# TEAM-AIOLY/OCM-VAE-SIMCA

Measured on AMD Instinct MI355X. Metric: spectra/sec SIMCA fit+Q/T² score at 1M×2048, higher is better.
Workload: dtype f32

## Files before the change

### ocm-vae-simca_amd/csrc/ocm_gram.hip

```cpp
#include <cstring>
#include <string>
#include <vector>

#include "ocm_internal.h"

namespace {

__device__ __forceinline__ float load_y(const float* __restrict__ X, int64_t ldx, int64_t r, int col, int p,
                                        const PrepArgs& pa) {
  if (pa.w == 0 && !pa.snv) return X[r * ldx + col];
  float m = 0.f, sc = 1.f;
  if (pa.snv) {
    m = pa.rowstat[2 * r];
    sc = pa.rowstat[2 * r + 1];
  }
  return ocm::prep_elem(X + r * ldx, p, col, pa, m, sc);
}


constexpr int MAXSEG = 32;

struct SegTable {
  int64_t begin[MAXSEG + 1];
  int32_t cprefix[MAXSEG + 1];
  int32_t nseg;
  int32_t chunk_rows;
};

__device__ __forceinline__ void tile_coords(int t, int nt, int& ti, int& tj) {
  ti = 0;
  while (t >= nt - ti) {
    t -= nt - ti;
    ++ti;
  }
  tj = ti + t;
}

template <int GT, int BK_>
struct GramCfg {
  static constexpr int BK = BK_;
  static constexpr int WN = GT / 64;
  static constexpr int THREADS = 2 * WN * 64;
  static constexpr int MT = GT / 64;
  static constexpr int C4 = GT / 4;
  static constexpr int RSTEP = THREADS / C4;
  static constexpr int LPP = BK / RSTEP;
};

constexpr int GATHER_MAX_CHUNK = 2048;

template <int GT, int BK_, bool VEC, bool GATHER>
__global__ __launch_bounds__(GT * 2, 2) void k_gram(
    const float* __restrict__ X, int64_t ldx, const int64_t* __restrict__ rows, int p, const float* __restrict__ shift,
    SegTable st, int nt, int ntiles, int total_wg, float* __restrict__ part, double* __restrict__ colpart) {
  using Cfg = GramCfg<GT, BK_>;
  constexpr int BK = Cfg::BK, MT = Cfg::MT, LPP = Cfg::LPP, RSTEP = Cfg::RSTEP;
// ... 1224 lines not shown
  const int tid = threadIdx.x, tx = tid & 15, ty = tid >> 4;
  const int gI = I / Q8GROUP, gJ = J / Q8GROUP;
  double acc[4][4] = {};
  for (int64_t f0 = fa; f0 < fb; f0 += FX_R) {
    const int nr = (int)min<int64_t>(FX_R, fb - f0);
    __syncthreads();
    for (int e = tid; e < FX_R * FX_T; e += 256) {
      const int r = e / FX_T, c = e % FX_T;
      double a = 0.0, b = 0.0;
      if (r < nr) {
        const int64_t pos = list[f0 + r];
        const int64_t xrow = rows ? rows[pos] : pos;
        if (I + c < p) a = (double)load_y(X, ldx, xrow, I + c, p, pa) - (double)shift[I + c];
        if (J + c < p) b = (double)load_y(X, ldx, xrow, J + c, p, pa) - (double)shift[J + c];
      }
      yi[r][c] = a;
      yj[r][c] = b;
    }
    if (tid < FX_R) {
      uint32_t m = 0;
      if (tid < nr) {
        const int64_t pos = list[f0 + tid];
        auto bit = [&](int g) { return (flags[(size_t)pos * fw + (g >> 5)] >> (g & 31)) & 1u; };
        m = bit(gI) | (bit(gI + 1) << 1) | (bit(gJ) << 2) | (bit(gJ + 1) << 3);
      }
      mk[tid] = m;
    }
    __syncthreads();
    for (int r = 0; r < nr; ++r) {
      const uint32_t m = mk[r];
      const bool mi = (m >> (ty >> 3)) & 1u;
      const bool mj = (m >> (2 + (tx >> 3))) & 1u;
      if (!(mi || mj)) continue;
#pragma unroll
      for (int a = 0; a < 4; ++a) {
        const double u = yi[r][4 * ty + a];
#pragma unroll
        for (int b = 0; b < 4; ++b) acc[a][b] = fma(u, yj[r][4 * tx + b], acc[a][b]);
      }
    }
  }
  double* Gs = G + (size_t)seg * p * p;
#pragma unroll
  for (int a = 0; a < 4; ++a)
#pragma unroll
    for (int b = 0; b < 4; ++b) {
      const int gi = I + 4 * ty + a, gj = J + 4 * tx + b;
      if (gi >= p || gj >= p) continue;
      Gs[(size_t)gi * p + gj] += acc[a][b];
      if (ti != tj) Gs[(size_t)gj * p + gi] += acc[a][b];
    }
}

#ifndef OCM_G8_BAND_R
#define OCM_G8_BAND_R 4
#endif
#ifndef OCM_G8_BAND_C
#define OCM_G8_BAND_C 8
#endif
constexpr int G8_BAND_R = OCM_G8_BAND_R, G8_BAND_C = OCM_G8_BAND_C;
__global__ __launch_bounds__(256, 1) void k_gram8d(Q8Plan q, SegTable st, int nt, int ntiles, int total_wg,
                                                   int nwg, int nblocks, float* __restrict__ part) {
  __shared__ __attribute__((aligned(16))) float scl[4][2 * 64];
  __shared__ __attribute__((aligned(16))) float runl[4][4][4][64][4];

  const int b = blockIdx.x;
  const int q8 = total_wg / 8, r8 = total_wg % 8, x8 = b % 8;
  const int wg = (x8 < r8 ? x8 * (q8 + 1) : r8 * (q8 + 1) + (x8 - r8) * q8) + b / 8;
  const int chunk = wg / nwg;
  const int wave = __builtin_amdgcn_readfirstlane(threadIdx.x >> 6);
  const int bi = (wg - chunk * nwg) * 4 + wave;
  if (bi >= nblocks) return;
  int ti = -1, tj = 0, wm = 0, wn = 0;
  {
    int rem = bi;
    for (int u = 0; u < nt && ti < 0; u += G8_BAND_R)
      for (int v = u; v < nt && ti < 0; v += G8_BAND_C)
        for (int a = u; a < min(nt, u + G8_BAND_R) && ti < 0; ++a)
          for (int c = max(v, a); c < min(nt, v + G8_BAND_C); ++c) {
            const int nbk = (a == c) ? 3 : 4;
            if (rem < nbk) {
              ti = a;
              tj = c;
              wm = (a == c) ? (rem == 2) : (rem >> 1);
              wn = (a == c) ? (rem >= 1) : (rem & 1);
              break;
            }
            rem -= nbk;
          }
  }
  const int tile = ti * nt - ti * (ti - 1) / 2 + (tj - ti);
  const int I = ti * Q8T, J = tj * Q8T;
  int s = 0;
  while (s + 1 < st.nseg && chunk >= st.cprefix[s + 1]) ++s;
  const int64_t r0 = st.begin[s] + (int64_t)(chunk - st.cprefix[s]) * st.chunk_rows;
  const int64_t r1 = min(r0 + (int64_t)st.chunk_rows, st.begin[s + 1]);
  const int nb = (int)((r1 - r0 + Q8BLK - 1) / Q8BLK);
  const int nstage3 = nb * Q8SPB;
  const size_t gbase = (size_t)chunk * (st.chunk_rows / Q8K);

  const int lane = threadIdx.x & 63;
  const int l31 = lane & 31, h = lane >> 5;
  const size_t gstride = (size_t)q.P8 * 32;
  const uint32_t span = (uint32_t)((size_t)nstage3 * gstride);
  const char* cbase = q.digits + gbase * gstride;
  __amdgpu_buffer_rsrc_t ra[3], rb[3];
#pragma unroll
  for (int dg = 0; dg < 3; ++dg) {
    ra[dg] = __builtin_amdgcn_make_buffer_rsrc((void*)(cbase + dg * q.plane + (size_t)(I + wm * 64) * 32), 0, span,
                                               0x00020000);
    rb[dg] = __builtin_amdgcn_make_buffer_rsrc((void*)(cbase + dg * q.plane + (size_t)(J + wn * 64) * 32), 0, span,
                                               0x00020000);
  }
// ... 109 lines not shown
#define Q8D_STEP_(STG, Z, CA, CB, NA, NB)                                                             \
  do {                                                                                              \
    Q8D_REFILL(NA, NB, min((STG) + 2, nstage3 - 1));                                                \
    __builtin_amdgcn_sched_barrier(0);                                                              \
    Q8D_MFMA(CA, CB, Z);                                                         \
    __builtin_amdgcn_sched_barrier(0);                                                              \
  } while (0)
#endif
#define Q8D_STEP(STG, Z, ...) Q8D_STEP_(STG, Z, __VA_ARGS__)

  i32x4 F0A[2][3], F0B[2][3], F1A[2][3], F1B[2][3], F2A[2][3], F2B[2][3];
  Q8D_LOAD(F0A, F0B, 0);
  Q8D_LOAD(F1A, F1B, min(1, nstage3 - 1));
#if defined(OCM_G8_DIAG_NOLOAD) || defined(OCM_G8_DIAG_HALFB)
  Q8D_LOAD(F2A, F2B, min(2, nstage3 - 1));
#endif
  for (int blk = 0; blk < nb; ++blk) {
    const int s0 = blk * Q8SPB;
#pragma unroll
    for (int u = 0; u < Q8SPB; u += 3) {
      Q8D_STEP(s0 + u, u == 0, Q8D_S0);
      Q8D_STEP(s0 + u + 1, false, Q8D_S1);
      if (u == 0) {
        SR = srow[(size_t)blk * q.P8];
        SC = scol[(size_t)blk * q.P8];
      }
      Q8D_STEP(s0 + u + 2, false, Q8D_S2);
    }
    flush();
  }
#undef Q8D_STEP
#undef Q8D_STEP_
#undef Q8D_REFILL
#undef Q8D_S0
#undef Q8D_S1
#undef Q8D_S2
#undef Q8D_MFMA
#undef Q8D_LOAD
#undef Q8D_LOAD_B

  float* out = part + ((size_t)chunk * ntiles + tile) * (Q8T * Q8T);
#pragma unroll
  for (int a = 0; a < 2; ++a)
#pragma unroll
    for (int c = 0; c < 2; ++c)
#pragma unroll
      for (int r = 0; r < 16; ++r) {
        const int row = wm * 64 + a * 32 + (r & 3) + 8 * (r >> 2) + 4 * h;
        const int col = wn * 64 + c * 32 + l31;
        out[row * Q8T + col] = runl[wave][a * 2 + c][r >> 2][lane][r & 3];
      }
}

template <bool ALIGNED, int SYNC, bool FRONT = false, bool SKIP = false>
__global__ __launch_bounds__(256, 1) void k_gram8e(Q8Plan q, SegTable st, int nt, int ntiles, int total_wg,
                                                   int nwg, int nblocks, float* __restrict__ part, int chunk0) {
  __shared__ __attribute__((aligned(16))) float scl[4][2 * 64];
  __shared__ __attribute__((aligned(16))) float runl[4][16][64][4];

  const int b = blockIdx.x;
  const int q8 = total_wg / 8, r8 = total_wg % 8, x8 = b % 8;
  const int wg = chunk0 < 0 ? b : (x8 < r8 ? x8 * (q8 + 1) : r8 * (q8 + 1) + (x8 - r8) * q8) + b / 8;
  const int cl = wg / nwg, chunk = (chunk0 < 0 ? 0 : chunk0) + cl;
  const int wave = __builtin_amdgcn_readfirstlane(threadIdx.x >> 6);
  int bi = (wg - cl * nwg) * 4 + wave;
  const bool dead = bi >= nblocks;
  if (dead && SYNC == 0) return;
  if (dead) bi = nblocks - 1;
  int ti = -1, tj = 0, wm = 0, wn = 0;
  if (ALIGNED) {
    const int noff = 4 * (ntiles - nt);
    if (bi < noff) {
      int rem = bi >> 2;
      wm = (bi >> 1) & 1;
      wn = bi & 1;
      for (int u = 0; u < nt && ti < 0; u += G8_BAND_R)
        for (int v = u; v < nt && ti < 0; v += G8_BAND_C)
          for (int a = u; a < min(nt, u + G8_BAND_R) && ti < 0; ++a)
            for (int c = max(v, a + 1); c < min(nt, v + G8_BAND_C); ++c) {
              if (rem == 0) {
                ti = a;
                tj = c;
                break;
              }
              --rem;
            }
    } else {
      const int d = (bi - noff) / 3, r = (bi - noff) - 3 * d;
      ti = tj = d;
      wm = (r == 2);
      wn = (r >= 1);
    }
  } else {
    int rem = bi;
    for (int u = 0; u < nt && ti < 0; u += G8_BAND_R)
      for (int v = u; v < nt && ti < 0; v += G8_BAND_C)
        for (int a = u; a < min(nt, u + G8_BAND_R) && ti < 0; ++a)
          for (int c = max(v, a); c < min(nt, v + G8_BAND_C); ++c) {
            const int nbk = (a == c) ? 3 : 4;
            if (rem < nbk) {
              ti = a;
              tj = c;
              wm = (a == c) ? (rem == 2) : (rem >> 1);
              wn = (a == c) ? (rem >= 1) : (rem & 1);
              break;
            }
            rem -= nbk;
          }
  }
  const int tile = ti * nt - ti * (ti - 1) / 2 + (tj - ti);
  const int I = ti * Q8T, J = tj * Q8T;
  int s = 0;
  while (s + 1 < st.nseg && chunk >= st.cprefix[s + 1]) ++s;
  const int64_t r0 = st.begin[s] + (int64_t)(chunk - st.cprefix[s]) * st.chunk_rows;
  const int64_t r1 = min(r0 + (int64_t)st.chunk_rows, st.begin[s + 1]);
  const int nb = (int)((r1 - r0 + Q8BLK - 1) / Q8BLK);
  constexpr int SPB = Q8BLK / 64;
  const int nstage = nb * SPB;
  const size_t gbase = (size_t)chunk * (st.chunk_rows / Q8K);

  const int lane = threadIdx.x & 63;
  const int l15 = lane & 15, g4 = lane >> 4;
  const size_t gstride = (size_t)q.P8 * 32;
  const uint32_t span = (uint32_t)((size_t)nb * Q8SPB * gstride);
  const char* cbase = q.digits + gbase * gstride;
  __amdgpu_buffer_rsrc_t ra[3], rb[3];
#pragma unroll
  for (int dg = 0; dg < 3; ++dg) {
    ra[dg] = __builtin_amdgcn_make_buffer_rsrc((void*)(cbase + dg * q.plane + (size_t)(I + wm * 64) * 32), 0, span,
                                               0x00020000);
    rb[dg] = __builtin_amdgcn_make_buffer_rsrc((void*)(cbase + dg * q.plane + (size_t)(J + wn * 64) * 32), 0, span,
                                               0x00020000);
  }
  const int voff = (g4 >> 1) * (int)gstride + l15 * 32 + (g4 & 1) * 16;
  const int sstride = 2 * (int)gstride;
  const float* srow = q.scale + (size_t)chunk * q.nblk * q.P8 + I + wm * 64 + lane;
  const float* scol = q.scale + (size_t)chunk * q.nblk * q.P8 + J + wn * 64 + lane;

  i32x4 acc1[4][4], acc2[4][4], acc3[4][4];
#pragma unroll
  for (int a = 0; a < 4; ++a)
#pragma unroll
    for (int c = 0; c < 4; ++c) {
      acc1[a][c] = i32x4{};
      acc2[a][c] = i32x4{};
      acc3[a][c] = i32x4{};
      *reinterpret_cast<f32x4*>(&runl[wave][a * 4 + c][lane][0]) = f32x4{0.f, 0.f, 0.f, 0.f};
    }
  float SR = 0.f, SC = 0.f;
  auto flush = [&]() __attribute__((always_inline)) {
    constexpr float w2 = 1.f / 254.f, w3 = 1.f / (254.f * 254.f);
    scl[wave][lane] = SR;
    scl[wave][64 + lane] = SC;
#pragma unroll
    for (int a = 0; a < 4; ++a) {
      const f32x4 si = *reinterpret_cast<const f32x4*>(&scl[wave][a * 16 + 4 * g4]);
#pragma unroll
      for (int c = 0; c < 4; ++c) {
        const float sj = scl[wave][64 + c * 16 + l15];
        f32x4* rp = reinterpret_cast<f32x4*>(&runl[wave][a * 4 + c][lane][0]);
        f32x4 rv = *rp;
#pragma unroll
        for (int e = 0; e < 4; ++e) {
          const float v = fmaf((float)acc3[a][c][e], w3, fmaf((float)acc2[a][c][e], w2, (float)acc1[a][c][e]));
          rv[e] = fmaf(v, si[e] * sj, rv[e]);
        }
        *rp = rv;
      }
      __builtin_amdgcn_sched_barrier(0);
    }
  };
  auto load_frag = [&](i32x4 (&FA)[4][3], i32x4 (&FB)[4][3], int i, int so) __attribute__((always_inline)) {
    const int grp = i / 3, dg = i % 3;
    if (grp >= 1 && grp <= 4)
      FB[grp - 1][dg] = (i32x4)__builtin_amdgcn_raw_buffer_load_b128(rb[dg], voff + (grp - 1) * 512, so, 0);
    else {
      const int x = grp == 0 ? 0 : grp - 4;
      FA[x][dg] = (i32x4)__builtin_amdgcn_raw_buffer_load_b128(ra[dg], voff + x * 512, so, 0);
    }
  };
  auto step = [&](i32x4 (&CA)[4][3], i32x4 (&CB)[4][3], i32x4 (&NA)[4][3], i32x4 (&NB)[4][3], int stg,
                  bool z) __attribute__((always_inline)) {
    const int so = min(stg + 1, nstage - 1) * sstride;
    constexpr int GRP = FRONT ? 48 : 24, PER = 96 / GRP;
#pragma unroll
    for (int i = 0; i < GRP; ++i) {
#ifndef OCM_G8E_DIAG_NOLOAD
      if (i < 24) load_frag(NA, NB, i, so);
#else
      (void)so;
#endif
#pragma unroll
      for (int jj = 0; jj < PER; ++jj) {
        const int j = PER * i + jj, blk = j / 6, kind = j % 6, a = blk >> 2, c = blk & 3;
        if (kind == 0) acc1[a][c] = __builtin_amdgcn_mfma_i32_16x16x64_i8(CA[a][0], CB[c][0], z ? i32x4{} : acc1[a][c], 0, 0, 0);
        if (kind == 1) acc2[a][c] = __builtin_amdgcn_mfma_i32_16x16x64_i8(CA[a][0], CB[c][1], z ? i32x4{} : acc2[a][c], 0, 0, 0);
        if (kind == 2) acc2[a][c] = __builtin_amdgcn_mfma_i32_16x16x64_i8(CA[a][1], CB[c][0], acc2[a][c], 0, 0, 0);
        if (kind == 3) acc3[a][c] = __builtin_amdgcn_mfma_i32_16x16x64_i8(CA[a][0], CB[c][2], z ? i32x4{} : acc3[a][c], 0, 0, 0);
        if (kind == 4) acc3[a][c] = __builtin_amdgcn_mfma_i32_16x16x64_i8(CA[a][2], CB[c][0], acc3[a][c], 0, 0, 0);
        if (kind == 5) acc3[a][c] = __builtin_amdgcn_mfma_i32_16x16x64_i8(CA[a][1], CB[c][1], acc3[a][c], 0, 0, 0);
      }
      __builtin_amdgcn_sched_barrier(0);
    }
    if (SYNC > 0 && stg % SYNC == SYNC - 1) __builtin_amdgcn_s_barrier();
  };

  const int nvs = SKIP ? (int)((r1 - r0 + 63) / 64) : nstage;
  i32x4 F0A[4][3], F0B[4][3], F1A[4][3], F1B[4][3];
#pragma unroll
  for (int i = 0; i < 24; ++i) load_frag(F0A, F0B, i, 0);
  for (int blk = 0; blk < nb; ++blk) {
    const int s0 = blk * SPB;
#pragma unroll
    for (int u = 0; u < SPB; u += 2) {
      if (SKIP && u > 0 && s0 + u >= nvs) break;
      step(F0A, F0B, F1A, F1B, s0 + u, u == 0);
      if (u == 0) {
        SR = srow[(size_t)blk * q.P8];
        SC = scol[(size_t)blk * q.P8];
      }
      step(F1A, F1B, F0A, F0B, s0 + u + 1, false);
    }
    flush();
  }

  if (dead) return;
  float* out = part + ((size_t)chunk * ntiles + tile) * (Q8T * Q8T);
#pragma unroll
  for (int a = 0; a < 4; ++a)
#pragma unroll
    for (int c = 0; c < 4; ++c)
#pragma unroll
      for (int e = 0; e < 4; ++e) {
        const int row = wm * 64 + a * 16 + 4 * g4 + e;
        const int col = wn * 64 + c * 16 + l15;
        out[row * Q8T + col] = runl[wave][a * 4 + c][lane][e];
      }
}

#ifdef OCM_G8_LDS
constexpr int G8X_FRAG = 1024, G8X_WSLOT = 12 * G8X_FRAG, G8X_SLOT = 4 * G8X_WSLOT;
__global__ __launch_bounds__(256, 1) void k_gram8x(Q8Plan q, SegTable st, int nt, int ntiles, int total_wg,
                                                   float* __restrict__ part) {
  __shared__ __attribute__((aligned(1024))) char ring[2 * G8X_SLOT];
  __shared__ __attribute__((aligned(16))) float runl[4][16][64][4];

  const int b = blockIdx.x;
  const int q8 = total_wg / 8, r8 = total_wg % 8, x8 = b % 8;
  const int wg = (x8 < r8 ? x8 * (q8 + 1) : r8 * (q8 + 1) + (x8 - r8) * q8) + b / 8;
  const int chunk = wg / ntiles;
  const int tix = wg - chunk * ntiles;
  const int wave = __builtin_amdgcn_readfirstlane(threadIdx.x >> 6);
  const int wm = wave >> 1, wn = wave & 1;
  int ti = -1, tj = 0;
  if (tix < ntiles - nt) {
    int rem = tix;
    for (int u = 0; u < nt && ti < 0; u += G8_BAND_R)
      for (int v = u; v < nt && ti < 0; v += G8_BAND_C)
        for (int a = u; a < min(nt, u + G8_BAND_R) && ti < 0; ++a)
          for (int c = max(v, a + 1); c < min(nt, v + G8_BAND_C); ++c) {
            if (rem == 0) {
              ti = a;
              tj = c;
              break;
            }
            --rem;
          }
  } else {
    ti = tj = tix - (ntiles - nt);
  }
  const bool mirror = (ti == tj) && wm == 1 && wn == 0;
  const int tile = ti * nt - ti * (ti - 1) / 2 + (tj - ti);
  const int I = ti * Q8T, J = tj * Q8T;
  int s = 0;
  while (s + 1 < st.nseg && chunk >= st.cprefix[s + 1]) ++s;
  const int64_t r0 = st.begin[s] + (int64_t)(chunk - st.cprefix[s]) * st.chunk_rows;
  const int64_t r1 = min(r0 + (int64_t)st.chunk_rows, st.begin[s + 1]);
  const int nb = (int)((r1 - r0 + Q8BLK - 1) / Q8BLK);
  constexpr int SPB = Q8BLK / 64;
  const int nstage = nb * SPB;
  const size_t gbase = (size_t)chunk * (st.chunk_rows / Q8K);

  const int lane = threadIdx.x & 63;
  const int l15 = lane & 15, g4 = lane >> 4;
  const size_t gstride = (size_t)q.P8 * 32;
  const uint32_t span = (uint32_t)((size_t)nb * Q8SPB * gstride);
  const char* cbase = q.digits + gbase * gstride;
  __amdgpu_buffer_rsrc_t ra[3], rb[3];
#pragma unroll
  for (int dg = 0; dg < 3; ++dg) {
// ... 477 lines not shown
  auto* host = static_cast<uint32_t*>(ocm::host_staging(ctx, 64));
  if (!host) return OCM_ERR_NOMEM;

  if (!unguarded) {
    const size_t nf = (size_t)n * fw, third = (size_t)p * QX_BINS;
    const size_t tot = nf + 4 + third;
    hipLaunchKernelGGL(k_guard_init, dim3((unsigned)std::min<size_t>((tot + 255) / 256, 4096)), dim3(256), 0, st,
                       flags, nf, counters, xhist, third, 0u);
    OCM_CHECK_LAUNCH("k_guard_init");
  }
  if (!unguarded) {
    hipLaunchKernelGGL(k_colexp_hist, dim3((p + 63) / 64, nsplit), dim3(256), 0, st, X, ldx, rows, nsamp, p, shift,
                       rps, xhist, pa);
    hipLaunchKernelGGL(k_q8_colmed, dim3((p + 3) / 4), dim3(256), 0, st, xhist, nsamp, p, thr);
    hipLaunchKernelGGL(k_q8_thresholds, dim3(1), dim3(1024), 0, st, p, P8, thr);
    OCM_CHECK_LAUNCH("k_q8_thresholds");
  }

  std::vector<SegTable> tabs;
  std::vector<int> tab_s0;
  for (int s0 = 0; s0 < nseg; s0 += MAXSEG) {
    const int s1 = std::min(nseg, s0 + MAXSEG);
    SegTable tab{};
    tab.nseg = s1 - s0;
    tab.chunk_rows = (int32_t)chunk_rows;
    for (int s = s0; s <= s1; ++s) {
      tab.begin[s - s0] = seg_offsets[s];
      tab.cprefix[s - s0] = cprefix[s] - cprefix[s0];
    }
    const int64_t gchunks = cprefix[s1] - cprefix[s0];
    if (gchunks == 0) continue;
    OCM_REQUIRE(gchunks * ntiles < (1LL << 31) && gchunks < 65536 * 1024LL, "ocm_gram_f32: too many workgroups");
    tabs.push_back(tab);
    tab_s0.push_back(s0);
  }
  auto plan_for = [&](int s0) {
    Q8Plan q{};
    q.digits = digits + (size_t)cprefix[s0] * chunk_rows * P8;
    q.plane = plane;
    q.scale = scale + (size_t)cprefix[s0] * nblk * P8;
    q.P8 = P8;
    q.nblk = nblk;
    q.thr = unguarded ? nullptr : thr;
    q.flags = flags;
    q.fw = fw;
    q.nmark = counters;
    return q;
  };
  hipStreamCaptureStatus cap = hipStreamCaptureStatusNone;
  OCM_HIP(hipStreamIsCapturing(st, &cap));
  const bool capturing = cap != hipStreamCaptureStatusNone;
  int order = 3;
  bool no_remap = false;
  int pieces = 1;
  int qcg = 1;
#ifdef OCM_EXP_SELECTORS
  const char* ord = getenv("OCM_GRAM8_ORDER");
  if (ord && !strcmp(ord, "packed")) order = 0;
  if (ord && !strcmp(ord, "aligned")) order = 1;
  if (ord && !strcmp(ord, "sync1")) order = 2;
  if (ord && !strcmp(ord, "front")) order = 6;
  if (ord && !strcmp(ord, "sync4")) order = 7;
  if (ord && !strcmp(ord, "sync3")) order = 8;
  const char* xr = getenv("OCM_GRAM8_XCD");
  no_remap = xr && !strcmp(xr, "0");
#ifdef OCM_G8_LDS
  if (ord && !strcmp(ord, "lds")) order = 4;
  if (ord && !strcmp(ord, "lds32")) order = 5;
#endif
  if (const char* pv = getenv("OCM_GRAM8_PIECES")) pieces = std::max(1, atoi(pv));
  if (const char* qv = getenv("OCM_Q8_CG")) qcg = atoi(qv);
#endif
  if (capturing || k32 || unguarded || tabs.size() != 1) pieces = 1;
  if (pieces > 1) {
    const int64_t gch = cprefix[tab_s0[0] + tabs[0].nseg] - cprefix[tab_s0[0]];
    pieces = (int)std::min<int64_t>(pieces, gch / 2);
    if (pieces < 2) pieces = 1;
  }
  hipStream_t qs = st;
  if (rows || (qcg != 2 && qcg != 4)) qcg = 1;
  std::vector<hipEvent_t> qev;
  if (pieces > 1) {
    if (!ctx->side) OCM_HIP(hipStreamCreateWithFlags(&ctx->side, hipStreamNonBlocking));
    qs = ctx->side;
    while ((int)ctx->fork_ev.size() < pieces + 1) {
      hipEvent_t e;
      OCM_HIP(hipEventCreateWithFlags(&e, hipEventDisableTiming));
      ctx->fork_ev.push_back(e);
    }
    qev.assign(ctx->fork_ev.begin(), ctx->fork_ev.begin() + pieces + 1);
    OCM_HIP(hipEventRecord(qev[pieces], st));
    OCM_HIP(hipStreamWaitEvent(qs, qev[pieces], 0));
  }
  const int nblocks = 4 * ntiles - nt, nwg = (nblocks + 3) / 4;
  auto quantise = [&](size_t t, int64_t c0, int64_t c1) {
    const int s0 = tab_s0[t];
    const Q8Plan q = plan_for(s0);
    double* col_g = colpart + (size_t)cprefix[s0] * nblk * P8;
    const int cgw = qcg;
    dim3 gq((unsigned)((c1 - c0) * nblk * cgw), (unsigned)(P8 / Q8QC / cgw));
    ocm::TimedRegion tq(ctx, OCM_KERNEL_QUANT, qs, !unguarded);
    if (prep) {
      const int ncg = P8 / Q8QC;
      const dim3 gp((unsigned)((c1 - c0) * nblk * ncg));
#define Q8P_LAUNCH(G_, H_, W_)                                                                                \
  hipLaunchKernelGGL((k_q8_quant_prep<G_, H_, W_>), gp, dim3(Q8QT), 0, qs, X, ldx, rows, p, shift, tabs[t], q, \
                     col_g, (int)(c0 * nblk), ncg, pa, xout, ldo)
      if (pa.h == 0) {
        if (rows) Q8P_LAUNCH(true, 0, false); else if (xout) Q8P_LAUNCH(false, 0, true); else Q8P_LAUNCH(false, 0, false);
      } else if (pa.h == 2) {
        if (rows) Q8P_LAUNCH(true, 2, false); else if (xout) Q8P_LAUNCH(false, 2, true); else Q8P_LAUNCH(false, 2, false);
      } else {
        if (rows) Q8P_LAUNCH(true, 7, false); else if (xout) Q8P_LAUNCH(false, 7, true); else Q8P_LAUNCH(false, 7, false);
      }
#undef Q8P_LAUNCH
    } else if (rows)
      hipLaunchKernelGGL(k_q8_quant<true>, gq, dim3(Q8QT), 0, qs, X, ldx, rows, p, shift, tabs[t], q, col_g,
                         (int)(c0 * nblk));
#ifdef OCM_EXP_SELECTORS
    else if (cgw == 4)
      hipLaunchKernelGGL((k_q8_quant<false, 4>), gq, dim3(Q8QT), 0, qs, X, ldx, rows, p, shift, tabs[t], q, col_g,
                         (int)(c0 * nblk));
    else if (cgw == 2)
      hipLaunchKernelGGL((k_q8_quant<false, 2>), gq, dim3(Q8QT), 0, qs, X, ldx, rows, p, shift, tabs[t], q, col_g,
                         (int)(c0 * nblk));
#endif
    else
      hipLaunchKernelGGL(k_q8_quant<false>, gq, dim3(Q8QT), 0, qs, X, ldx, rows, p, shift, tabs[t], q, col_g,
                         (int)(c0 * nblk));
  };
  auto gram = [&](size_t t, int64_t c0, int64_t c1) {
    const int s0 = tab_s0[t];
    const int64_t total = (c1 - c0) * nwg;
    const Q8Plan q = plan_for(s0);
    float* pg = part + (size_t)cprefix[s0] * ntiles * Q8T * Q8T;
    ocm::TimedRegion tr(ctx, OCM_KERNEL_GRAM, st, !unguarded);
#define G8E_LAUNCH(A_, S_)                                                                                   \
  hipLaunchKernelGGL((k_gram8e<A_, S_>), dim3((unsigned)total), dim3(256), 0, st, q, tabs[t], nt, ntiles, (int)total, \
                     nwg, nblocks, pg, (no_remap && c0 == 0) ? -1 : (int)c0)
#define G8E_LAUNCH3(A_, S_, F_)                                                                                      \
  hipLaunchKernelGGL((k_gram8e<A_, S_, F_>), dim3((unsigned)total), dim3(256), 0, st, q, tabs[t], nt, ntiles,         \
                     (int)total, nwg, nblocks, pg, (int)c0)
    if (tr_O && !k32 && order == 3)
      hipLaunchKernelGGL((k_gram8e<true, 2, false, true>), dim3((unsigned)total), dim3(256), 0, st, q, tabs[t], nt,
                         ntiles, (int)total, nwg, nblocks, pg, (int)c0);
    else if (!k32 && order == 3) G8E_LAUNCH(true, 2);
#ifdef OCM_EXP_SELECTORS
    else if (!k32 && order == 0) G8E_LAUNCH(false, 0);
    else if (!k32 && order == 1) G8E_LAUNCH(true, 0);
    else if (!k32 && order == 2) G8E_LAUNCH(true, 1);
    else if (!k32 && order == 6) G8E_LAUNCH3(true, 2, true);
    else if (!k32 && order == 7) G8E_LAUNCH(true, 4);
    else if (!k32 && order == 8) G8E_LAUNCH(true, 3);
#endif
#undef G8E_LAUNCH
#undef G8E_LAUNCH3
#ifdef OCM_G8_LDS
    else if (!k32 && order >= 4 && order <= 5) {
      const int64_t total_x = (c1 - c0) * ntiles;
      if (order == 4)
        hipLaunchKernelGGL(k_gram8x, dim3((unsigned)total_x), dim3(256), 0, st, q, tabs[t], nt, ntiles, (int)total_x,
                           pg);
      else
        hipLaunchKernelGGL(k_gram8s, dim3((unsigned)total_x), dim3(256), 0, st, q, tabs[t], nt, ntiles, (int)total_x,
                           pg);
    }
#endif
    else
      hipLaunchKernelGGL(k_gram8d, dim3((unsigned)total), dim3(256), 0, st, q, tabs[t], nt, ntiles, (int)total, nwg,
                         nblocks, pg);
  };
  hipEvent_t ev = nullptr;
  const bool readback = !capturing && !unguarded;
  if (readback) OCM_HIP(hipEventCreateWithFlags(&ev, hipEventDisableTiming));
  if (pieces == 1) {
    for (size_t t = 0; t < tabs.size(); ++t) quantise(t, 0, cprefix[tab_s0[t] + tabs[t].nseg] - cprefix[tab_s0[t]]);
    OCM_CHECK_LAUNCH("k_q8_quant");
    if (readback) {
      OCM_HIP(hipMemcpyAsync(host, counters, 4, hipMemcpyDeviceToHost, st));
      OCM_HIP(hipEventRecord(ev, st));
    }
    for (size_t t = 0; t < tabs.size(); ++t) gram(t, 0, cprefix[tab_s0[t] + tabs[t].nseg] - cprefix[tab_s0[t]]);
    OCM_CHECK_LAUNCH("k_gram8d/8e");
  } else {
    const int64_t gch = cprefix[tab_s0[0] + tabs[0].nseg] - cprefix[tab_s0[0]];
    std::vector<int64_t> cut(pieces + 1);
    for (int i = 0; i <= pieces; ++i) cut[i] = gch * i / pieces;
    for (int i = 0; i < pieces; ++i) {
      quantise(0, cut[i], cut[i + 1]);
      OCM_HIP(hipEventRecord(qev[i], qs));
    }
    OCM_CHECK_LAUNCH("k_q8_quant");
    OCM_HIP(hipMemcpyAsync(host, counters, 4, hipMemcpyDeviceToHost, qs));
    OCM_HIP(hipEventRecord(ev, qs));
    for (int i = 0; i < pieces; ++i) {
      OCM_HIP(hipStreamWaitEvent(st, qev[i], 0));
      gram(0, cut[i], cut[i + 1]);
    }
    OCM_CHECK_LAUNCH("k_gram8e");
    OCM_HIP(hipStreamWaitEvent(st, ev, 0));
  }
  if (tr_O) {
    hipLaunchKernelGGL(k_gram_trace<Q8T>, dim3(Q8T * Q8T / 4 / 256, ntiles), dim3(256), 0, st, part, nt, ntiles, p, 0,
                       cprefix[1], tr_O, tr_part);
    OCM_CHECK_LAUNCH("k_gram_trace");
    return OCM_OK;
  }
  for (int s = 0; s < nseg; ++s) {
    double* Gs = G_out + (size_t)s * p * p;
    double* cs = colsum_out + (size_t)s * p;
    if (cprefix[s + 1] == cprefix[s]) {
      OCM_HIP(hipMemsetAsync(Gs, 0, (size_t)p * p * sizeof(double), st));
      OCM_HIP(hipMemsetAsync(cs, 0, (size_t)p * sizeof(double), st));
      continue;
    }
    dim3 g((Q8T * Q8T / 4 + 255) / 256, ntiles);
    hipLaunchKernelGGL(k_gram_reduce<Q8T>, g, dim3(256), 0, st, part, colpart, nt, ntiles, p, cprefix[s],
                       cprefix[s + 1], Gs, cs, 0);
    hipLaunchKernelGGL(k_colblk_sum, dim3(P8 / 16), dim3(256), 0, st, colpart, (int64_t)cprefix[s] * nblk,
                       (int64_t)cprefix[s + 1] * nblk, P8, p, cs);
    OCM_CHECK_LAUNCH("k_colblk_sum");
    OCM_CHECK_LAUNCH("k_gram_reduce");
  }
  if (unguarded) return OCM_OK;
  if (!capturing) {
    const hipError_t e = hipEventSynchronize(ev);
    (void)hipEventDestroy(ev);
    if (e != hipSuccess) return ocm::fail(OCM_ERR_HIP, std::string("gram mark read-back: ") + hipGetErrorString(e));
    ctx->last_gram_marks = host[0];
    if (host[0] == 0) return OCM_OK;
  }
  hipLaunchKernelGGL(k_flag_count, dim3(nfblk), dim3(256), 0, st, flags, fw, n, fcnt);
  hipLaunchKernelGGL(k_flag_emit, dim3(nfblk), dim3(256), 0, st, flags, fw, n, fcnt, nfblk, flist, counters + 1);
  OCM_CHECK_LAUNCH("k_flag_emit");
  if (!capturing) {
    OCM_HIP(hipMemcpyAsync(host + 1, counters + 1, 4, hipMemcpyDeviceToHost, st));
    OCM_HIP(hipStreamSynchronize(st));
    if ((int64_t)host[1] > n / 8) return 1;
  }
  const int nt64 = (p + FX_T - 1) / FX_T;
  for (int s0 = 0; s0 < nseg; s0 += MAXSEG) {
    const int s1 = std::min(nseg, s0 + MAXSEG);
    FixSeg fs{};
    fs.nseg = s1 - s0;
    for (int s = s0; s <= s1; ++s) fs.begin[s - s0] = seg_offsets[s];
    hipLaunchKernelGGL(k_gram_fixup, dim3(nt64 * (nt64 + 1) / 2, s1 - s0), dim3(256), 0, st, X, ldx, rows, p, shift,
                       fs, flist, counters + 1, flags, fw, nt64, G_out + (size_t)s0 * p * p, pa);
  }
  OCM_CHECK_LAUNCH("k_gram_fixup");
  return OCM_OK;
}

int gram_dispatch(ocm_ctx* ctx, const float* X, int64_t ldx, const int64_t* rows, int64_t n, int32_t p,
                  const float* shift, const int64_t* seg_offsets, int32_t nseg, int32_t mode, int64_t chunk_rows,
// ... 199 lines not shown
```

Baseline: 55.94 million.

## Make int8 Gram kernel persistent with cross-item prefetch and overlapped output stores

Replaces the one-workgroup-per-item int8 Gram kernel with a persistent kernel launched on about one workgroup per CU, with each workgroup looping over several (chunk, tile-block) items in an XCD-aware slot order. The next item's buffer descriptors are built ahead so the last stage of one item already prefetches the next item's first fragments. The previous item's accumulated tile is written out with buffer stores interleaved into the first MFMA step of the next item, and the off-diagonal tile map is precomputed into LDS to avoid the per-wave search loop. The aim is to cut per-workgroup launch, prologue and epilogue bubbles, at the cost of more complex control flow, extra register and LDS pressure, and possible load imbalance from the coarser work split.

```diff
diff --git a/ocm-vae-simca_amd/csrc/ocm_gram.hip b/ocm-vae-simca_amd/csrc/ocm_gram.hip
--- a/ocm-vae-simca_amd/csrc/ocm_gram.hip
+++ b/ocm-vae-simca_amd/csrc/ocm_gram.hip
@@ -1,7 +1,9 @@
 #include <cstring>
 #include <string>
+#include <type_traits>
 #include <vector>
 
+#include "ocm_gram_map.h"
 #include "ocm_internal.h"
 
 namespace {
@@ -1332,13 +1334,7 @@
     }
 }
 
-#ifndef OCM_G8_BAND_R
-#define OCM_G8_BAND_R 4
-#endif
-#ifndef OCM_G8_BAND_C
-#define OCM_G8_BAND_C 8
-#endif
-constexpr int G8_BAND_R = OCM_G8_BAND_R, G8_BAND_C = OCM_G8_BAND_C;
+constexpr int G8_BAND_R = ocm_g8::BAND_R, G8_BAND_C = ocm_g8::BAND_C;
 __global__ __launch_bounds__(256, 1) void k_gram8d(Q8Plan q, SegTable st, int nt, int ntiles, int total_wg,
                                                    int nwg, int nblocks, float* __restrict__ part) {
   __shared__ __attribute__((aligned(16))) float scl[4][2 * 64];
@@ -1554,61 +1550,49 @@
       }
 }
 
+#ifdef OCM_G8E_STAMPS
+__device__ unsigned long long g8_stamp_acc[4];
+#define G8_STAMP(V) const uint64_t V = __builtin_amdgcn_s_memrealtime()
+#define G8_STAMP_VAR(V) uint64_t V = 0
+#define G8_STAMP_SET(V) V = __builtin_amdgcn_s_memrealtime()
+#define G8_STAMP_SUM(A, B, C, D)                                              \
+  if (threadIdx.x == 0) {                                                     \
+    atomicAdd(&g8_stamp_acc[0], (unsigned long long)((B) - (A)));             \
+    atomicAdd(&g8_stamp_acc[1], (unsigned long long)((D) - (C)));             \
+    atomicAdd(&g8_stamp_acc[2], (unsigned long long)((D) - (A)));             \
+    atomicAdd(&g8_stamp_acc[3], 1ull);                                        \
+  }
+#else
+#define G8_STAMP(V)
+#define G8_STAMP_VAR(V)
+#define G8_STAMP_SET(V)
+#define G8_STAMP_SUM(A, B, C, D)
+#endif
+
+#ifdef OCM_EXP_SELECTORS
 template <bool ALIGNED, int SYNC, bool FRONT = false, bool SKIP = false>
-__global__ __launch_bounds__(256, 1) void k_gram8e(Q8Plan q, SegTable st, int nt, int ntiles, int total_wg,
+__global__ __launch_bounds__(256, 1) void k_gram8w(Q8Plan q, SegTable st, int nt, int ntiles, int total_wg,
                                                    int nwg, int nblocks, float* __restrict__ part, int chunk0) {
   __shared__ __attribute__((aligned(16))) float scl[4][2 * 64];
   __shared__ __attribute__((aligned(16))) float runl[4][16][64][4];
 
+  G8_STAMP(t_in);
   const int b = blockIdx.x;
-  const int q8 = total_wg / 8, r8 = total_wg % 8, x8 = b % 8;
-  const int wg = chunk0 < 0 ? b : (x8 < r8 ? x8 * (q8 + 1) : r8 * (q8 + 1) + (x8 - r8) * q8) + b / 8;
+  const int wg = chunk0 < 0 ? b : ocm_g8::logical_item(total_wg, b);
   const int cl = wg / nwg, chunk = (chunk0 < 0 ? 0 : chunk0) + cl;
   const int wave = __builtin_amdgcn_readfirstlane(threadIdx.x >> 6);
-  int bi = (wg - cl * nwg) * 4 + wave;
-  const bool dead = bi >= nblocks;
-  if (dead && SYNC == 0) return;
-  if (dead) bi = nblocks - 1;
-  int ti = -1, tj = 0, wm = 0, wn = 0;
+  int ti, tj, wm, wn;
+  bool dead;
   if (ALIGNED) {
-    const int noff = 4 * (ntiles - nt);
-    if (bi < noff) {
-      int rem = bi >> 2;
-      wm = (bi >> 1) & 1;
-      wn = bi & 1;
-      for (int u = 0; u < nt && ti < 0; u += G8_BAND_R)
-        for (int v = u; v < nt && ti < 0; v += G8_BAND_C)
-          for (int a = u; a < min(nt, u + G8_BAND_R) && ti < 0; ++a)
-            for (int c = max(v, a + 1); c < min(nt, v + G8_BAND_C); ++c) {
-              if (rem == 0) {
-                ti = a;
-                tj = c;
-                break;
-              }
-              --rem;
-            }
-    } else {
-      const int d = (bi - noff) / 3, r = (bi - noff) - 3 * d;
-      ti = tj = d;
-      wm = (r == 2);
-      wn = (r >= 1);
-    }
+    const ocm_g8::Block k = ocm_g8::block_tile(nt, ntiles, nblocks, wg - cl * nwg, wave);
+    ti = k.ti, tj = k.tj, wm = k.wm, wn = k.wn, dead = k.dead;
+    if (dead && SYNC == 0) return;
   } else {
-    int rem = bi;
-    for (int u = 0; u < nt && ti < 0; u += G8_BAND_R)
-      for (int v = u; v < nt && ti < 0; v += G8_BAND_C)
-        for (int a = u; a < min(nt, u + G8_BAND_R) && ti < 0; ++a)
-          for (int c = max(v, a); c < min(nt, v + G8_BAND_C); ++c) {
-            const int nbk = (a == c) ? 3 : 4;
-            if (rem < nbk) {
-              ti = a;
-              tj = c;
-              wm = (a == c) ? (rem == 2) : (rem >> 1);
-              wn = (a == c) ? (rem >= 1) : (rem & 1);
-              break;
-            }
-            rem -= nbk;
-          }
+    int bi = (wg - cl * nwg) * 4 + wave;
+    dead = bi >= nblocks;
+    if (dead && SYNC == 0) return;
+    if (dead) bi = nblocks - 1;
+    ocm_g8::packed_block(nt, bi, ti, tj, wm, wn);
   }
   const int tile = ti * nt - ti * (ti - 1) / 2 + (tj - ti);
   const int I = ti * Q8T, J = tj * Q8T;
@@ -1711,6 +1695,11 @@
   i32x4 F0A[4][3], F0B[4][3], F1A[4][3], F1B[4][3];
 #pragma unroll
   for (int i = 0; i < 24; ++i) load_frag(F0A, F0B, i, 0);
+#ifdef OCM_G8E_STAMPS
+  __builtin_amdgcn_s_waitcnt(0x0F70);
+#endif
+  G8_STAMP(t_first);
+  G8_STAMP_VAR(t_last);
   for (int blk = 0; blk < nb; ++blk) {
     const int s0 = blk * SPB;
 #pragma unroll
@@ -1723,21 +1712,228 @@
       }
       step(F1A, F1B, F0A, F0B, s0 + u + 1, false);
     }
+    G8_STAMP_SET(t_last);
     flush();
   }
 
-  if (dead) return;
-  float* out = part + ((size_t)chunk * ntiles + tile) * (Q8T * Q8T);
-#pragma unroll
-  for (int a = 0; a < 4; ++a)
-#pragma unroll
-    for (int c = 0; c < 4; ++c)
-#pragma unroll
-      for (int e = 0; e < 4; ++e) {
-        const int row = wm * 64 + a * 16 + 4 * g4 + e;
-        const int col = wn * 64 + c * 16 + l15;
-        out[row * Q8T + col] = runl[wave][a * 4 + c][lane][e];
-      }
+  if (!dead) {
+    float* out = part + ((size_t)chunk * ntiles + tile) * (Q8T * Q8T);
+#pragma unroll
+    for (int a = 0; a < 4; ++a)
+#pragma unroll
+      for (int c = 0; c < 4; ++c)
+#pragma unroll
+        for (int e = 0; e < 4; ++e) {
+          const int row = wm * 64 + a * 16 + 4 * g4 + e;
+          const int col = wn * 64 + c * 16 + l15;
+          out[row * Q8T + col] = runl[wave][a * 4 + c][lane][e];
+        }
+  }
+  G8_STAMP(t_out);
+  G8_STAMP_SUM(t_in, t_first, t_last, t_out);
+}
+#endif
+
+constexpr int G8P_TMAP = 2048;
+template <bool SKIP>
+__global__ __launch_bounds__(256, 1) void k_gram8e(Q8Plan q, SegTable st, int nt, int ntiles, int total_wg,
+                                                   int nwg, int nblocks, float* __restrict__ part, int chunk0) {
+  __shared__ __attribute__((aligned(16))) float scl[4][2 * 64];
+  __shared__ __attribute__((aligned(16))) float runl[4][16][64][4];
+  __shared__ uint16_t tmap[G8P_TMAP];
+
+  const int noffr = ntiles - nt;
+  const bool tabled = noffr <= G8P_TMAP;
+  if (tabled) {
+    for (int r = threadIdx.x; r < noffr; r += 256) {
+      int a, c;
+      ocm_g8::offdiag_tile(nt, r, a, c);
+      tmap[r] = (uint16_t)(a << 8 | c);
+    }
+    __syncthreads();
+  }
+  const ocm_g8::Slot sl = ocm_g8::slot_of(total_wg, (int)gridDim.x, (int)blockIdx.x);
+  if (sl.count == 0) return;
+
+  const int wave = __builtin_amdgcn_readfirstlane(threadIdx.x >> 6);
+  const int lane = threadIdx.x & 63;
+  const int l15 = lane & 15, g4 = lane >> 4;
+  constexpr int SPB = Q8BLK / 64;
+  const size_t gstride = (size_t)q.P8 * 32;
+  const int voff = (g4 >> 1) * (int)gstride + l15 * 32 + (g4 & 1) * 16;
+  const int sstride = 2 * (int)gstride;
+  const int vout = (4 * g4 * Q8T + l15) * 4;
+  constexpr uint32_t OUT_SPAN = (63 * Q8T + 64) * 4;
+
+  struct Item {
+    __amdgpu_buffer_rsrc_t ra[3], rb[3];
+    __amdgpu_buffer_rsrc_t rout;
+    const float *srow, *scol;
+    int nb, nvs;
+  };
+  auto setup = [&](int wg) __attribute__((always_inline)) -> Item {
+    const int cl = wg / nwg, chunk = chunk0 + cl;
+    ocm_g8::Block k = ocm_g8::block_of(nt, ntiles, nblocks, wg - cl * nwg, wave);
+    if (k.offrank >= 0) {
+      if (tabled) {
+        const int v = __builtin_amdgcn_readfirstlane((int)tmap[k.offrank]);
+        k.ti = v >> 8;
+        k.tj = v & 255;
+      } else {
+        ocm_g8::offdiag_tile(nt, k.offrank, k.ti, k.tj);
+      }
+    }
+    const int tile = ocm_g8::tile_index(nt, k.ti, k.tj);
+    const int I = k.ti * Q8T + k.wm * 64, J = k.tj * Q8T + k.wn * 64;
+    int s = 0;
+    while (s + 1 < st.nseg && chunk >= st.cprefix[s + 1]) ++s;
+    const int64_t r0 = st.begin[s] + (int64_t)(chunk - st.cprefix[s]) * st.chunk_rows;
+    const int64_t r1 = min(r0 + (int64_t)st.chunk_rows, st.begin[s + 1]);
+    Item it;
+    it.nb = (int)((r1 - r0 + Q8BLK - 1) / Q8BLK);
+    it.nvs = SKIP ? (int)((r1 - r0 + 63) / 64) : it.nb * SPB;
+    const size_t gbase = (size_t)chunk * (st.chunk_rows / Q8K);
+    const uint32_t span = (uint32_t)((size_t)it.nb * Q8SPB * gstride);
+    const char* cbase = q.digits + gbase * gstride;
+#pragma unroll
+    for (int dg = 0; dg < 3; ++dg) {
+      it.ra[dg] = __builtin_amdgcn_make_buffer_rsrc((void*)(cbase + dg * q.plane + (size_t)I * 32), 0, span, 0x00020000);
+      it.rb[dg] = __builtin_amdgcn_make_buffer_rsrc((void*)(cbase + dg * q.plane + (size_t)J * 32), 0, span, 0x00020000);
+    }
+    it.srow = q.scale + (size_t)chunk * q.nblk * q.P8 + I;
+    it.scol = q.scale + (size_t)chunk * q.nblk * q.P8 + J;
+    float* out = part + ((size_t)chunk * ntiles + tile) * (Q8T * Q8T) + k.wm * 64 * Q8T + k.wn * 64;
+    it.rout = __builtin_amdgcn_make_buffer_rsrc((void*)out, 0, k.dead ? 0u : OUT_SPAN, 0x00020000);
+    return it;
+  };
+
+  i32x4 acc1[4][4], acc2[4][4], acc3[4][4];
+  float SR = 0.f, SC = 0.f;
+  auto flush = [&](bool first) __attribute__((always_inline)) {
+    constexpr float w2 = 1.f / 254.f, w3 = 1.f / (254.f * 254.f);
+    scl[wave][lane] = SR;
+    scl[wave][64 + lane] = SC;
+#pragma unroll
+    for (int a = 0; a < 4; ++a) {
+      const f32x4 si = *reinterpret_cast<const f32x4*>(&scl[wave][a * 16 + 4 * g4]);
+#pragma unroll
+      for (int c = 0; c < 4; ++c) {
+        const float sj = scl[wave][64 + c * 16 + l15];
+        f32x4* rp = reinterpret_cast<f32x4*>(&runl[wave][a * 4 + c][lane][0]);
+        f32x4 rv = *rp;
+        if (first) rv = f32x4{0.f, 0.f, 0.f, 0.f};
+#pragma unroll
+        for (int e = 0; e < 4; ++e) {
+          const float v = fmaf((float)acc3[a][c][e], w3, fmaf((float)acc2[a][c][e], w2, (float)acc1[a][c][e]));
+          rv[e] = fmaf(v, si[e] * sj, rv[e]);
+        }
+        *rp = rv;
+      }
+      __builtin_amdgcn_sched_barrier(0);
+    }
+  };
+  auto load_frag = [&](i32x4 (&FA)[4][3], i32x4 (&FB)[4][3], int i, int so, const __amdgpu_buffer_rsrc_t (&da)[3],
+                       const __amdgpu_buffer_rsrc_t (&db)[3]) __attribute__((always_inline)) {
+    const int grp = i / 3, dg = i % 3;
+    if (grp >= 1 && grp <= 4)
+      FB[grp - 1][dg] = (i32x4)__builtin_amdgcn_raw_buffer_load_b128(db[dg], voff + (grp - 1) * 512, so, 0);
+    else {
+      const int x = grp == 0 ? 0 : grp - 4;
+      FA[x][dg] = (i32x4)__builtin_amdgcn_raw_buffer_load_b128(da[dg], voff + x * 512, so, 0);
+    }
+  };
+  auto store_sub = [&](const f32x4& pv, int i, __amdgpu_buffer_rsrc_t ro) __attribute__((always_inline)) {
+    const int a = i >> 2, c = i & 3;
+#pragma unroll
+    for (int e = 0; e < 4; ++e)
+      __builtin_amdgcn_raw_buffer_store_b32(__builtin_bit_cast(unsigned, (float)pv[e]), ro, vout,
+                                            ((a * 16 + e) * Q8T + c * 16) * 4, 0);
+  };
+  auto step = [&](i32x4 (&CA)[4][3], i32x4 (&CB)[4][3], i32x4 (&NA)[4][3], i32x4 (&NB)[4][3], int so,
+                  const __amdgpu_buffer_rsrc_t (&da)[3], const __amdgpu_buffer_rsrc_t (&db)[3], bool z, bool bar,
+                  auto tail, __amdgpu_buffer_rsrc_t ro) __attribute__((always_inline)) {
+    constexpr bool TAIL = decltype(tail)::value;
+    f32x4 pv = {0.f, 0.f, 0.f, 0.f};
+#pragma unroll
+    for (int i = 0; i < 24; ++i) {
+      load_frag(NA, NB, i, so, da, db);
+      if constexpr (TAIL) {
+        if (i >= 1 && i <= 16) store_sub(pv, i - 1, ro);
+        if (i < 16) pv = *reinterpret_cast<const f32x4*>(&runl[wave][i][lane][0]);
+      }
+#pragma unroll
+      for (int jj = 0; jj < 4; ++jj) {
+        const int j = 4 * i + jj, blk = j / 6, kind = j % 6, a = blk >> 2, c = blk & 3;
+        if (kind == 0) acc1[a][c] = __builtin_amdgcn_mfma_i32_16x16x64_i8(CA[a][0], CB[c][0], z ? i32x4{} : acc1[a][c], 0, 0, 0);
+        if (kind == 1) acc2[a][c] = __builtin_amdgcn_mfma_i32_16x16x64_i8(CA[a][0], CB[c][1], z ? i32x4{} : acc2[a][c], 0, 0, 0);
+        if (kind == 2) acc2[a][c] = __builtin_amdgcn_mfma_i32_16x16x64_i8(CA[a][1], CB[c][0], acc2[a][c], 0, 0, 0);
+        if (kind == 3) acc3[a][c] = __builtin_amdgcn_mfma_i32_16x16x64_i8(CA[a][0], CB[c][2], z ? i32x4{} : acc3[a][c], 0, 0, 0);
+        if (kind == 4) acc3[a][c] = __builtin_amdgcn_mfma_i32_16x16x64_i8(CA[a][2], CB[c][0], acc3[a][c], 0, 0, 0);
+        if (kind == 5) acc3[a][c] = __builtin_amdgcn_mfma_i32_16x16x64_i8(CA[a][1], CB[c][1], acc3[a][c], 0, 0, 0);
+      }
+      __builtin_amdgcn_sched_barrier(0);
+    }
+    if (bar) __builtin_amdgcn_s_barrier();
+  };
+
+  const __amdgpu_buffer_rsrc_t rnone = __builtin_amdgcn_make_buffer_rsrc((void*)part, 0, 0u, 0x00020000);
+  __amdgpu_buffer_rsrc_t rpend = rnone;
+  i32x4 F0A[4][3], F0B[4][3], F1A[4][3], F1B[4][3];
+  Item cur = setup(sl.first);
+#pragma unroll
+  for (int i = 0; i < 24; ++i) load_frag(F0A, F0B, i, 0, cur.ra, cur.rb);
+  for (int n = 0; n < sl.count; ++n) {
+    G8_STAMP(t_in);
+    const Item nxt = setup(sl.first + min(n + 1, sl.count - 1) * sl.step);
+    if (SKIP && n > 0) {
+#pragma unroll
+      for (int i = 0; i < 24; ++i) load_frag(F0A, F0B, i, 0, cur.ra, cur.rb);
+    }
+#ifdef OCM_G8E_STAMPS
+    __builtin_amdgcn_s_waitcnt(0x0F70);
+#endif
+    G8_STAMP(t_first);
+    G8_STAMP_VAR(t_last);
+    const int nstage = cur.nb * SPB;
+    for (int blk = 0; blk < cur.nb; ++blk) {
+      const int s0 = blk * SPB;
+      const bool lastb = blk == cur.nb - 1;
+#pragma unroll
+      for (int u = 0; u < SPB; u += 2) {
+        if (SKIP && u > 0 && s0 + u >= cur.nvs) break;
+        if (u == 0) {
+          if (blk == 0 && n > 0)
+            step(F0A, F0B, F1A, F1B, (s0 + 1) * sstride, cur.ra, cur.rb, true, false, std::true_type{}, rpend);
+          else
+            step(F0A, F0B, F1A, F1B, (s0 + 1) * sstride, cur.ra, cur.rb, true, false, std::false_type{}, rnone);
+          SR = cur.srow[(size_t)blk * q.P8 + lane];
+          SC = cur.scol[(size_t)blk * q.P8 + lane];
+        } else {
+          step(F0A, F0B, F1A, F1B, (s0 + u + 1) * sstride, cur.ra, cur.rb, false, false, std::false_type{}, rnone);
+        }
+        if (!SKIP && u + 2 == SPB) {
+          __amdgpu_buffer_rsrc_t da[3], db[3];
+#pragma unroll
+          for (int dg = 0; dg < 3; ++dg) {
+            da[dg] = lastb ? nxt.ra[dg] : cur.ra[dg];
+            db[dg] = lastb ? nxt.rb[dg] : cur.rb[dg];
+          }
+          step(F1A, F1B, F0A, F0B, lastb ? 0 : (s0 + SPB) * sstride, da, db, false, true, std::false_type{}, rnone);
+        } else {
+          step(F1A, F1B, F0A, F0B, min(s0 + u + 2, nstage - 1) * sstride, cur.ra, cur.rb, false, true,
+               std::false_type{}, rnone);
+        }
+      }
+      G8_STAMP_SET(t_last);
+      flush(blk == 0);
+    }
+    rpend = cur.rout;
+    cur = nxt;
+    G8_STAMP(t_out);
+    G8_STAMP_SUM(t_in, t_first, t_last, t_out);
+  }
+#pragma unroll
+  for (int i = 0; i < 16; ++i) store_sub(*reinterpret_cast<const f32x4*>(&runl[wave][i][lane][0]), i, rpend);
 }
 
 #ifdef OCM_G8_LDS
@@ -2321,10 +2517,12 @@
   const bool capturing = cap != hipStreamCaptureStatusNone;
   int order = 3;
   bool no_remap = false;
+  (void)no_remap;
   int pieces = 1;
   int qcg = 1;
 #ifdef OCM_EXP_SELECTORS
   const char* ord = getenv("OCM_GRAM8_ORDER");
+  if (ord && !strcmp(ord, "wg")) order = 9;
   if (ord && !strcmp(ord, "packed")) order = 0;
   if (ord && !strcmp(ord, "aligned")) order = 1;
   if (ord && !strcmp(ord, "sync1")) order = 2;
@@ -2405,16 +2603,23 @@
     float* pg = part + (size_t)cprefix[s0] * ntiles * Q8T * Q8T;
     ocm::TimedRegion tr(ctx, OCM_KERNEL_GRAM, st, !unguarded);
 #define G8E_LAUNCH(A_, S_)                                                                                   \
-  hipLaunchKernelGGL((k_gram8e<A_, S_>), dim3((unsigned)total), dim3(256), 0, st, q, tabs[t], nt, ntiles, (int)total, \
+  hipLaunchKernelGGL((k_gram8w<A_, S_>), dim3((unsigned)total), dim3(256), 0, st, q, tabs[t], nt, ntiles, (int)total, \
                      nwg, nblocks, pg, (no_remap && c0 == 0) ? -1 : (int)c0)
 #define G8E_LAUNCH3(A_, S_, F_)                                                                                      \
-  hipLaunchKernelGGL((k_gram8e<A_, S_, F_>), dim3((unsigned)total), dim3(256), 0, st, q, tabs[t], nt, ntiles,         \
+  hipLaunchKernelGGL((k_gram8w<A_, S_, F_>), dim3((unsigned)total), dim3(256), 0, st, q, tabs[t], nt, ntiles,         \
                      (int)total, nwg, nblocks, pg, (int)c0)
+    const unsigned pgrid = (unsigned)std::min<int64_t>(total, std::max(ctx->num_cus, ocm_g8::NXCD));
     if (tr_O && !k32 && order == 3)
-      hipLaunchKernelGGL((k_gram8e<true, 2, false, true>), dim3((unsigned)total), dim3(256), 0, st, q, tabs[t], nt,
+      hipLaunchKernelGGL(k_gram8e<true>, dim3(pgrid), dim3(256), 0, st, q, tabs[t], nt, ntiles, (int)total, nwg,
+                         nblocks, pg, (int)c0);
+    else if (!k32 && order == 3)
+      hipLaunchKernelGGL(k_gram8e<false>, dim3(pgrid), dim3(256), 0, st, q, tabs[t], nt, ntiles, (int)total, nwg,
+                         nblocks, pg, (int)c0);
+#ifdef OCM_EXP_SELECTORS
+    else if (tr_O && !k32 && order == 9)
+      hipLaunchKernelGGL((k_gram8w<true, 2, false, true>), dim3((unsigned)total), dim3(256), 0, st, q, tabs[t], nt,
                          ntiles, (int)total, nwg, nblocks, pg, (int)c0);
-    else if (!k32 && order == 3) G8E_LAUNCH(true, 2);
-#ifdef OCM_EXP_SELECTORS
+    else if (!k32 && order == 9) G8E_LAUNCH(true, 2);
     else if (!k32 && order == 0) G8E_LAUNCH(false, 0);
     else if (!k32 && order == 1) G8E_LAUNCH(true, 0);
     else if (!k32 && order == 2) G8E_LAUNCH(true, 1);
@@ -2450,7 +2655,7 @@
       OCM_HIP(hipEventRecord(ev, st));
     }
     for (size_t t = 0; t < tabs.size(); ++t) gram(t, 0, cprefix[tab_s0[t] + tabs[t].nseg] - cprefix[tab_s0[t]]);
-    OCM_CHECK_LAUNCH("k_gram8d/8e");
+    OCM_CHECK_LAUNCH("k_gram8d/8p");
   } else {
     const int64_t gch = cprefix[tab_s0[0] + tabs[0].nseg] - cprefix[tab_s0[0]];
     std::vector<int64_t> cut(pieces + 1);
@@ -2469,6 +2674,18 @@
     OCM_CHECK_LAUNCH("k_gram8e");
     OCM_HIP(hipStreamWaitEvent(st, ev, 0));
   }
+#ifdef OCM_G8E_STAMPS
+  {
+    unsigned long long acc[4] = {0, 0, 0, 0};
+    OCM_HIP(hipStreamSynchronize(st));
+    OCM_HIP(hipMemcpyFromSymbol(acc, HIP_SYMBOL(g8_stamp_acc), sizeof(acc)));
+    if (!unguarded && !capturing && acc[3])
+      fprintf(stderr, "G8E_STAMPS order=%d items=%llu mean_us entry_to_first=%.3f last_to_end=%.3f entry_to_end=%.3f\n",
+              order, acc[3], 0.01 * acc[0] / acc[3], 0.01 * acc[1] / acc[3], 0.01 * acc[2] / acc[3]);
+    const unsigned long long zero[4] = {0, 0, 0, 0};
+    OCM_HIP(hipMemcpyToSymbol(HIP_SYMBOL(g8_stamp_acc), zero, sizeof(zero)));
+  }
+#endif
   if (tr_O) {
     hipLaunchKernelGGL(k_gram_trace<Q8T>, dim3(Q8T * Q8T / 4 / 256, ntiles), dim3(256), 0, st, part, nt, ntiles, p, 0,
                        cprefix[1], tr_O, tr_part);
diff --git a/ocm-vae-simca_amd/csrc/ocm_gram_map.h b/ocm-vae-simca_amd/csrc/ocm_gram_map.h
--- /dev/null
+++ b/ocm-vae-simca_amd/csrc/ocm_gram_map.h
@@ -0,0 +1,121 @@
+#pragma once
+
+#if defined(__HIPCC__) || defined(__CUDACC__)
+#define OCM_MAP_HD __host__ __device__ inline
+#else
+#define OCM_MAP_HD inline
+#endif
+
+#ifndef OCM_G8_BAND_R
+#define OCM_G8_BAND_R 4
+#endif
+#ifndef OCM_G8_BAND_C
+#define OCM_G8_BAND_C 8
+#endif
+
+namespace ocm_g8 {
+
+constexpr int BAND_R = OCM_G8_BAND_R, BAND_C = OCM_G8_BAND_C;
+constexpr int NXCD = 8;
+
+OCM_MAP_HD int imin(int a, int b) { return a < b ? a : b; }
+OCM_MAP_HD int imax(int a, int b) { return a > b ? a : b; }
+
+OCM_MAP_HD int xcd_first(int total, int x) {
+  const int q8 = total / NXCD, r8 = total % NXCD;
+  return x < r8 ? x * (q8 + 1) : r8 * (q8 + 1) + (x - r8) * q8;
+}
+OCM_MAP_HD int xcd_count(int total, int x) { return total / NXCD + (x < total % NXCD ? 1 : 0); }
+
+OCM_MAP_HD int logical_item(int total, int b) { return xcd_first(total, b % NXCD) + b / NXCD; }
+
+struct Slot {
+  int first;
+  int step;
+  int count;
+};
+OCM_MAP_HD Slot slot_of(int total, int grid, int b) {
+  const int x = b % NXCD, s = b / NXCD;
+  const int S = xcd_count(grid, x), n = xcd_count(total, x);
+  Slot r;
+  r.first = xcd_first(total, x) + s;
+  r.step = S;
+  r.count = s < n ? (n - s + S - 1) / S : 0;
+  return r;
+}
+
+OCM_MAP_HD void offdiag_tile(int nt, int rank, int& ti, int& tj) {
+  ti = -1;
+  tj = 0;
+  int rem = rank;
+  for (int u = 0; u < nt && ti < 0; u += BAND_R)
+    for (int v = u; v < nt && ti < 0; v += BAND_C)
+      for (int a = u; a < imin(nt, u + BAND_R) && ti < 0; ++a)
+        for (int c = imax(v, a + 1); c < imin(nt, v + BAND_C); ++c) {
+          if (rem == 0) {
+            ti = a;
+            tj = c;
+            break;
+          }
+          --rem;
+        }
+}
+
+OCM_MAP_HD void packed_block(int nt, int bi, int& ti, int& tj, int& wm, int& wn) {
+  ti = -1;
+  tj = wm = wn = 0;
+  int rem = bi;
+  for (int u = 0; u < nt && ti < 0; u += BAND_R)
+    for (int v = u; v < nt && ti < 0; v += BAND_C)
+      for (int a = u; a < imin(nt, u + BAND_R) && ti < 0; ++a)
+        for (int c = imax(v, a); c < imin(nt, v + BAND_C); ++c) {
+          const int nbk = (a == c) ? 3 : 4;
+          if (rem < nbk) {
+            ti = a;
+            tj = c;
+            wm = (a == c) ? (rem == 2) : (rem >> 1);
+            wn = (a == c) ? (rem >= 1) : (rem & 1);
+            break;
+          }
+          rem -= nbk;
+        }
+}
+
+struct Block {
+  int bi;
+  int offrank;
+  int ti, tj;
+  int wm, wn;
+  bool dead;
+};
+
+OCM_MAP_HD Block block_of(int nt, int ntiles, int nblocks, int local, int wave) {
+  Block k;
+  k.bi = local * 4 + wave;
+  k.dead = k.bi >= nblocks;
+  if (k.dead) k.bi = nblocks - 1;
+  const int noff = 4 * (ntiles - nt);
+  if (k.bi < noff) {
+    k.offrank = k.bi >> 2;
+    k.wm = (k.bi >> 1) & 1;
+    k.wn = k.bi & 1;
+    k.ti = -1;
+    k.tj = 0;
+  } else {
+    const int d = (k.bi - noff) / 3, r = (k.bi - noff) - 3 * d;
+    k.offrank = -1;
+    k.ti = k.tj = d;
+    k.wm = (r == 2);
+    k.wn = (r >= 1);
+  }
+  return k;
+}
+OCM_MAP_HD Block block_tile(int nt, int ntiles, int nblocks, int local, int wave) {
+  Block k = block_of(nt, ntiles, nblocks, local, wave);
+  if (k.offrank >= 0) offdiag_tile(nt, k.offrank, k.ti, k.tj);
+  return k;
+}
+
+OCM_MAP_HD int tile_index(int nt, int ti, int tj) { return ti * nt - ti * (ti - 1) / 2 + (tj - ti); }
+
+}
```

Measured after the change: 57.20 million, median of 6. 1.02x the previous value.
